# deepmarkpy/aware

Hardware: AMD Instinct MI355X
Metric: waveform-seconds/sec through embed->attack->detect; BER vs reference (higher is better)
Workload: dtype f32 accumulation on the 16-bit MFMA pipe; conv-block GEMMs: every f32 operand scaled by a power of two and carried as TWO binary16 terms (within one f32 ulp of the operand, rms 2^-24.5), 3 partial products, the l_a*l_b term (<= 2^-22) dropped -- gemm_h2.hip: error level of an f32 dot product (agains

## Files before the change

### aware_amd/_lib.py

```python
from __future__ import annotations

import ctypes as C
import glob
import os
import subprocess

_HERE = os.path.dirname(os.path.abspath(__file__))
LIB_PATH = os.environ.get("AWARE_HIP_LIB") or os.path.join(_HERE, "libaware_hip.so")
CSRC = os.path.join(_HERE, "csrc")
SOURCES = ["capi.hip", "dsp_kernels.hip", "dsp_stream.hip", "seam_kernels.hip", "detector_kernels.hip", "gemm_x3.hip", "gemm_h2.hip", "attack_kernels.hip", "stft_any.hip", "loop_any.hip", "stoi_kernels.hip", "loop_attack_kernels.hip", "loop_reverb_kernels.hip", "loop_speed_kernels.hip", "loop_stretch_kernels.hip", "loop_pitch_kernels.hip", "loop_pv_kernels.hip", "loop_delete_kernels.hip", "loop_filter_kernels.hip", "sync_kernels.hip", "loop_mix_kernels.hip", "loop_gain_kernels.hip", "speed_search_kernels.hip", "scan_kernels.hip", "viterbi_kernels.hip"]

AWARE_OK = 0
ERRORS = {-1: "bad argument", -2: "unsupported configuration", -3: "HIP runtime error", -4: "workspace too small"}


class AwareHipError(RuntimeError):
    pass


def build_library(force: bool = False, verbose: bool = False) -> str:
    from concurrent.futures import ThreadPoolExecutor
    hdrs = glob.glob(os.path.join(CSRC, "*.hpp")) + glob.glob(os.path.join(CSRC, "*.h")) + [
        os.path.join(_HERE, "..", "include", "aware_hip.h")]
    hdr_t = max(os.path.getmtime(h) for h in hdrs)
# ... 135 lines not shown
    "aware_opt_clamp_step": (_i, [_i, _vp, _vp, _vp, _vp, _vp, _vp, _sz, C.POINTER(C.c_float), C.POINTER(C.c_float), _vp]),
    "aware_embed_begin": (_i, [_vp, _vp, _vp, _vp]),
    "aware_embed_iterate": (_i, [_vp, _i, _vp]),
    "aware_embed_profile": (_i, [_vp, _i, _i, _vp, _vp, _vp]),
    "aware_embed_gradient": (_i, [_vp, _vp, _vp]),
    "aware_embed_finish": (_i, [_vp, _vp, _vp, _vp]),
    "aware_embed_buffer": (_vp, [_vp, _i]),
    "aware_pcm_quantize": (_i, [_vp, _vp, _vp, _vp, _i, _i, _i, _vp, _vp]),
    "aware_waveform_normalize": (_i, [_vp, _vp, _vp, _vp, _i, _i, _vp, _vp]),
    "aware_upfirdn": (_i, [_vp, _vp, _vp, _vp, _vp, _vp, _i, _i, _vp, _i, _i, _i, _i, _vp]),
    "aware_iir": (_i, [_vp, _vp, _vp, _i, _i, _vp, _i, _vp, _vp, _vp, _i, _i, _vp, _vp]),
    "aware_decimate_interp": (_i, [_vp, _vp, _vp, _i, _i, _i, _vp, _vp]),
    "aware_segment_cut": (_i, [_vp, _vp, _vp, _vp, _vp, _vp, _vp, _i, _i, _i, _vp]),
    "aware_phase_vocoder": (_i, [_vp, _vp, _vp, _vp, _i, C.c_double, _vp]),
    "aware_snr": (_i, [_vp, _vp, _vp, _vp, _vp, _i, _vp, _vp]),
    "aware_stoi_create": (_i, [C.POINTER(_vp)]),
    "aware_stoi_destroy": (None, [_vp]),
    "aware_stoi_band_edges": (_i, [_vp, _pi, _pi]),
    "aware_stoi_frames": (_i, [_i]),
    "aware_stoi_workspace_bytes": (_sz, [_i, _i, C.c_longlong]),
    "aware_stoi": (_i, [_vp, _vp, _vp, _vp, _vp, _vp, _i, _i, C.c_longlong, _vp, _vp, _vp, _sz, _vp]),
    "aware_gaussian_noise": (_i, [_vp, _vp, _vp, _vp, _i, _i, _vp, _f, _vp, _vp]),
    "aware_spectral_quantize": (_i, [_vp, _i, _f, _f, _vp]),
    "aware_spectral_quantize_bwd": (_i, [_vp, _vp, _vp, _i, _f, _f, _vp]),
    "aware_gemm_nt_variant": (_i, [_vp, _i, _vp, _i, _vp, _vp, _i, _i, _i, _i, _i, _vp]),
    "aware_x3_packed_bytes": (_sz, [_i, _i]),
    "aware_x3_pack": (_i, [_vp, _i, _i, _vp]),
    "aware_gemm_clip": (_i, [_vp, _i, _vp, _i, _vp, _vp, _vp, _i, _i, _i, _i, _i, _i, _vp, _vp, _i, _vp]),
    "aware_gemm_clip_last": (_i, [_vp, _i, _vp, _vp, _vp, _i, _i, _i, _i, _i, _vp, _vp, _vp, _i, _vp]),
    "aware_gemm_clip_h2_workspace_bytes": (_sz, [_i, _i, _i]),
    "aware_gemm_clip_h2": (_i, [_vp, _i, _vp, _i, _vp, _vp, _i, _i, _i, _i, _i, _i, _vp, _vp, _vp, _vp, _i, _vp, _vp, _sz, _vp]),
    "aware_gemm_clip_h2_tile": (_i, [_vp, _i, _vp, _i, _vp, _vp, _i, _i, _i, _i, _i, _i, _vp, _vp, _vp, _vp, _i, _vp, _vp, _sz, _i,
                                     _vp]),
    "aware_gemm_nt": (_i, [_vp, _i, _vp, _i, _vp, _vp, _i, _i, _i, _i, _vp]),
}

_lib = None


def load_library():
    global _lib
    if _lib is not None:
        return _lib
    if not os.path.exists(LIB_PATH):
        raise AwareHipError(
            f"{LIB_PATH} is missing: build it with `python -c 'import __graft_entry__ as g; g.build()'` "
            "(hipcc --offload-arch=gfx950).  aware_amd has no CPU fallback.")
    import torch
    lib = C.CDLL(LIB_PATH)
    for name, (res, args) in SIGNATURES.items():
        fn = getattr(lib, name)
        fn.restype = res
        fn.argtypes = args
    _lib = lib
    return lib


def check(rc: int, what: str = ""):
    if rc != AWARE_OK:
        lib = load_library()
        detail = lib.aware_last_hip_error().decode() if rc == -3 else ""
        raise AwareHipError(f"{what}: {ERRORS.get(rc, rc)} {detail}".strip())


def require_gpu():
    import torch
# ... 4 lines not shown
```

### aware_amd/csrc/capi.hip

```cpp
#include <hip/hip_runtime.h>
#include <math.h>
#include <cmath>
#include <stdio.h>
#include <stdlib.h>
#include <string.h>
#include <string>
#include <algorithm>
#include <vector>

#include "../../include/aware_hip.h"
#include "common.hpp"
#include "kernels.h"
#define AWARE_LOOP_CF cf
#include "loop_chain.hpp"

using namespace aware;

static thread_local std::string g_last_err;

#define HIPCHK(expr)                                                                  \
    do {                                                                              \
        hipError_t _e = (expr);                                                       \
        if (_e != hipSuccess) {                                                       \
            g_last_err = std::string(#expr) + ": " + hipGetErrorString(_e);           \
// ... 2923 lines not shown

extern "C" size_t aware_gemm_clip_h2_workspace_bytes(int B, int N, int K) {
    return (B > 0 && N > 0 && K > 0) ? h2_packed_bytes(N, K) + (size_t)B * 64 * sizeof(float) * 2 + 1024 : 0;
}
extern "C" int aware_gemm_clip_h2(const float* A, int lda, const float* Bt, int ldb, const float* bias, float* C, int ldc, int B,
                                  int Tp, int N, int K, int epi, float* rstd_io, const float* act, const void* lastpk, float* zpart,
                                  int CL, float* amax_out, void* workspace, size_t workspace_bytes, void* stream) {
    return aware_gemm_clip_h2_tile(A, lda, Bt, ldb, bias, C, ldc, B, Tp, N, K, epi, rstd_io, act, lastpk, zpart, CL, amax_out,
                                   workspace, workspace_bytes, 0, stream);
}
extern "C" int aware_gemm_clip_h2_tile(const float* A, int lda, const float* Bt, int ldb, const float* bias, float* C, int ldc,
                                       int B, int Tp, int N, int K, int epi, float* rstd_io, const float* act, const void* lastpk,
                                       float* zpart, int CL, float* amax_out, void* workspace, size_t workspace_bytes, int tile,
                                       void* stream) {
    if (tile < 0 || tile > 2) return AWARE_E_BADARG;
    if (!A || !Bt || !C || !workspace || B < 1 || Tp < 1 || Tp > 128 || epi < 0 || epi > 2 || (ldb & 3)) return AWARE_E_BADARG;
    if (epi != 0 && !rstd_io) return AWARE_E_BADARG;
    if (epi == 2 && !act) return AWARE_E_BADARG;
    const int nwm = (Tp + 31) / 32;
    if (!gemm_clip_h2_supported(nwm, N, K, lda) || N % 16) return AWARE_E_BADARG;
    if (tile == 2 && !gemm_clip_h2_wide_supported(nwm, N, K, lda)) return AWARE_E_UNSUPPORTED;
    if (workspace_bytes < aware_gemm_clip_h2_workspace_bytes(B, N, K)) return AWARE_E_WORKSPACE;
    hipStream_t st = (hipStream_t)stream;
    Carver c(workspace, workspace_bytes);
    void* pk = c.take<char>(h2_packed_bytes(N, K));
    float* amax = c.take<float>((size_t)B * 64);
    launch_h2_pack(Bt, ldb, N, K, pk, st);
    launch_clip_amax(A, lda, K, 32 * nwm, B, amax, st);
    launch_gemm_clip_h2(A, lda, pk, amax, amax_out, bias, C, ldc, B, nwm, Tp, N, K, epi, rstd_io, act, st,
                        (epi == 1 && lastpk && zpart) ? lastpk : nullptr, zpart, CL, tile == 2 ? 2 : 1);
    LAUNCHCHK();
    return AWARE_OK;
}

extern "C" int aware_gemm_nt(const float* A, int lda, const float* Bt, int ldb, const float* bias, float* C, int ldc,
                             int M, int N, int K, void* stream) {
    if (!A || !Bt || !C || M < 1 || N < 1 || K < 4 || (K & 3) || (lda & 3) || (ldb & 3)) return AWARE_E_BADARG;
    launch_gemm_nt(A, lda, Bt, ldb, bias, C, ldc, M, N, K, (hipStream_t)stream);
    LAUNCHCHK();
    return AWARE_OK;
}
```

### aware_amd/csrc/conv_block.hpp

```cpp
#pragma once
#include <hip/hip_runtime.h>
#include "split_bf16.hpp"

namespace aware {

constexpr int kConvFrag = 1024;

template <class P, int RG, int EPI>
constexpr int conv_block_lds_bytes() {
    constexpr int stage = 2 * 2 * P::kTerms * 2 * RG * kConvFrag;
    constexpr int last = 32 * RG * 132 * 4 > 8 * RG * 3 * kConvFrag ? 32 * RG * 132 * 4 : 8 * RG * 3 * kConvFrag;
    return (EPI == X3_FWD_LAST && last > stage) ? last : stage;
}

constexpr int conv_tile_width(int NT, int NW) { return 16 * NT * NW; }

__host__ __device__ inline int conv_slab_group(int tiles_n, int width, int K, int weight_bytes) {
    int sg = (int)(3355443u / (unsigned)(width * K * weight_bytes));
    sg = sg < 1 ? 1 : (sg > tiles_n ? tiles_n : sg);
    while (tiles_n % sg) --sg;
    return sg;
}

template <class P, int RG, int EPI, int NT = 1, int NW = 8>
__device__ __forceinline__ void conv_block_uniform(const float* __restrict__ A, int lda, const u32x4* __restrict__ Bpk,
                                                   const float* __restrict__ binv, const float* __restrict__ amax_in,
                                                   float* __restrict__ amax_out, const float* __restrict__ bias,
                                                   float* __restrict__ C, int ldc, int Tp, int N, int K, int tiles_n, int ntiles,
                                                   float* __restrict__ rstd_io, const float* __restrict__ act,
                                                   const u32x4* __restrict__ Lpk, float* __restrict__ zpart, int CL, int Mrows) {
    constexpr int MT = 2 * RG;
    constexpr int MH = RG;
    constexpr int FRAG = kConvFrag;
    constexpr int W = conv_tile_width(NT, NW);
    static_assert(NT == 1 || P::kScaled, "the row-major PLAIN epilogue of the unscaled format is written for one column tile");
    static_assert(W % 128 == 0 && (NW == 8 || NW == 4), "FWD_LAST works on whole 128-column slabs with 4 or 8 waves");
    __shared__ __attribute__((aligned(16))) unsigned char lds[conv_block_lds_bytes<P, RG, EPI>()];

    int id = blockIdx.x;
    int clip, slab;
    if ((ntiles & 7) == 0) {
        const int x = id & 7, j = id >> 3, R = ntiles >> 3;
        const int nclip = R / tiles_n;
        if (nclip * tiles_n == R && nclip > 0) {
            const int sg = conv_slab_group(tiles_n, W, K, P::kWeightBytes);
            const int per_group = nclip * sg;
            const int grp = j / per_group, r = j % per_group;
            clip = x * nclip + r / sg;
            slab = grp * sg + r % sg;
        } else {
            id = x * R + j;
            clip = id / tiles_n;
            slab = id % tiles_n;
        }
    } else {
        clip = id / tiles_n;
        slab = id % tiles_n;
    }
    const int bm = clip * 32 * RG;
    const int bn = slab * W;
    const int tid = threadIdx.x, lane = tid & 63, wave = tid >> 6;
    const int r16 = lane & 15, kg = lane >> 4;
    const int col0 = bn + wave * (16 * NT) + r16;

    float ascale = 1.f, ainv = 1.f;
    if constexpr (P::kScaled) {
        float am = lane < (K >> 4) ? amax_in[(size_t)clip * 64 + lane] : 0.f;
#pragma unroll
        for (int o = 32; o > 0; o >>= 1) am = fmaxf(am, __shfl_xor(am, o));
        ascale = __uint_as_float(__builtin_amdgcn_readfirstlane(__float_as_uint(P::scale_for(am))));
    }

    f32x4 acc[MT][NT];
    const int row_limit = (!P::kScaled && EPI == X3_PLAIN) ? min(32 * RG, Mrows - bm) : 32 * RG;
    if constexpr (NT == 1 && NW == 8) P::template tile_gemm<RG>(A, lda, Bpk, K, bm, bn, lds, acc, row_limit, ascale);
    else P::template tile_gemm<RG, NT, NW>(A, lda, Bpk, K, bm, bn, lds, acc, row_limit, ascale);

    if constexpr (P::kScaled) ainv = P::pow2_inverse(ascale);
    const float invT = 1.0f / (float)Tp;
    if constexpr (!P::kScaled && EPI == X3_PLAIN) {
        if ((ldc & 3) == 0) {
            float (*T)[132] = reinterpret_cast<float (*)[132]>(lds);
            const float bv = bias ? bias[col0] : 0.f;
            __syncthreads();
#pragma unroll
            for (int m = 0; m < MT; ++m)
#pragma unroll
                for (int e = 0; e < 4; ++e) T[16 * m + 4 * kg + e][16 * wave + r16] = acc[m][0][e] + bv;
            __syncthreads();
            const int c4 = (lane & 31) * 4, rr = 2 * wave + (lane >> 5);
#pragma unroll
            for (int j = 0; j < MT; ++j) {
                const int row = rr + 16 * j;
                float4 o = *reinterpret_cast<const float4*>(&T[row][c4]);
                if (row >= Tp) o = make_float4(0.f, 0.f, 0.f, 0.f);
                if (bm + row < Mrows) *reinterpret_cast<float4*>(C + (size_t)(bm + row) * ldc + bn + c4) = o;
            }
            return;
        }
    }
#pragma unroll
    for (int n = 0; n < NT; ++n) {
    const int col = col0 + 16 * n;
    float bcol = 1.f;
    if constexpr (P::kScaled) bcol = binv[col];
    float omax = 0.f;
    if (EPI == X3_PLAIN) {
        const float bv = bias ? bias[col] : 0.f;
#pragma unroll
        for (int m = 0; m < MT; ++m)
#pragma unroll
            for (int e = 0; e < 4; ++e) {
                const int row = m * 16 + 4 * kg + e;
                const float o = row < Tp ? fmaf(acc[m][n][e] * ainv, bcol, bv) : 0.f;
                omax = fmaxf(omax, fabsf(o));
                if (P::kScaled || bm + row < Mrows) C[(size_t)(bm + row) * ldc + col] = o;
            }
    } else if (EPI == X3_FWD || EPI == X3_FWD_LAST) {
        const float bv = bias ? bias[col] : 0.f;
        float s = 0.f;
#pragma unroll
        for (int m = 0; m < MT; ++m)
#pragma unroll
            for (int e = 0; e < 4; ++e) {
                const int row = m * 16 + 4 * kg + e;
                acc[m][n][e] = fmaf(acc[m][n][e] * ainv, bcol, bv);
                if (row < Tp) s += acc[m][n][e];
            }
        s += __shfl_xor(s, 16);
        s += __shfl_xor(s, 32);
        const float mean = s * invT;
        auto centre = [&](float x) {
            if constexpr (P::kScaled) return fmaf(-invT, s, x);
            else return x - mean;
        };
        float qq = 0.f;
#pragma unroll
        for (int m = 0; m < MT; ++m)
#pragma unroll
            for (int e = 0; e < 4; ++e) {
                const int row = m * 16 + 4 * kg + e;
                if (row < Tp) {
                    const float d = centre(acc[m][n][e]);
                    if constexpr (P::kScaled) qq = fmaf(d, d, qq);
                    else qq += d * d;
                }
            }
        qq += __shfl_xor(qq, 16);
        qq += __shfl_xor(qq, 32);
        const float rs = 1.0f / sqrtf(qq * invT + 1e-5f);
        if (kg == 0) rstd_io[(size_t)clip * N + col] = rs;
#pragma unroll
        for (int m = 0; m < MT; ++m)
#pragma unroll
            for (int e = 0; e < 4; ++e) {
                const int row = m * 16 + 4 * kg + e;
                const float u = centre(acc[m][n][e]) * rs;
                const float o = row < Tp ? (u > 0.f ? u : 0.2f * u) : 0.f;
                acc[m][n][e] = o;
                omax = fmaxf(omax, fabsf(o));
                C[(size_t)(bm + row) * ldc + col] = o;
            }
    } else {
        const float rs = rstd_io[(size_t)clip * N + col];
        float s1 = 0.f, s2 = 0.f;
        float u[MT][4];
#pragma unroll
        for (int m = 0; m < MT; ++m)
#pragma unroll
            for (int e = 0; e < 4; ++e) {
                const int row = m * 16 + 4 * kg + e;
                const float av = act[(size_t)(bm + row) * ldc + col];
                const bool valid = row < Tp;
                const float uv = valid ? (av > 0.f ? av : av * 5.0f) : 0.f;
                const float du = valid ? acc[m][n][e] * ainv * bcol * (av > 0.f ? 1.f : 0.2f) : 0.f;
                acc[m][n][e] = du;
                u[m][e] = uv;
                s1 += du;
                s2 += du * uv;
            }
        s1 += __shfl_xor(s1, 16);
        s1 += __shfl_xor(s1, 32);
        s2 += __shfl_xor(s2, 16);
        s2 += __shfl_xor(s2, 32);
        const float m1 = s1 * invT, m2 = s2 * invT;
#pragma unroll
        for (int m = 0; m < MT; ++m)
#pragma unroll
            for (int e = 0; e < 4; ++e) {
                const int row = m * 16 + 4 * kg + e;
                const float o = row < Tp ? rs * (acc[m][n][e] - m1 - u[m][e] * m2) : 0.f;
                omax = fmaxf(omax, fabsf(o));
                C[(size_t)(bm + row) * ldc + col] = o;
            }
    }
    if constexpr (P::kScaled) {
        if (amax_out) {
#pragma unroll
            for (int o = 32; o > 0; o >>= 1) omax = fmaxf(omax, __shfl_xor(omax, o));
            if (lane == 0) amax_out[(size_t)clip * 64 + (col >> 4)] = omax;
        }
    }
    }
    if (EPI == X3_FWD_LAST) {
        const int KS2L = N >> 5, ncl = (CL + 15) >> 4;
        constexpr int UH = 8 / NW;
        constexpr int WS = 8 / NT;
        const int tq = NW == 8 ? wave >> 1 : wave, mh0 = NW == 8 ? wave & 1 : 0;
        float* const T = reinterpret_cast<float*>(lds);
        constexpr int TP = 132;
#pragma unroll
        for (int sl = 0; sl < W / 128; ++sl) {
        const int slab128 = (bn >> 7) + sl;
        bf16x8 bl[3][3];
#pragma unroll
        for (int n = 0; n < 3; ++n)
            if (n < ncl) {
#pragma unroll
                for (int p = 0; p < 3; ++p)
                    bl[n][p] = __builtin_bit_cast(bf16x8, Lpk[(((size_t)n * KS2L + 4 * slab128 + tq) * 3 + p) * 64 + lane]);
            }
        __syncthreads();
        if (wave / WS == sl) {
#pragma unroll
            for (int n = 0; n < NT; ++n)
#pragma unroll
                for (int m = 0; m < MT; ++m)
#pragma unroll
                    for (int e = 0; e < 4; ++e)
                        T[(16 * m + 4 * kg + e) * TP + 16 * ((wave % WS) * NT + n) + r16] = acc[m][n][e];
        }
        __syncthreads();
        f32x4 zt[UH * MH][3];
#pragma unroll
        for (int mm = 0; mm < UH * MH; ++mm) {
#pragma unroll
            for (int n = 0; n < 3; ++n) zt[mm][n] = f32x4{0.f, 0.f, 0.f, 0.f};
            const float* src = T + (16 * (mh0 * MH + mm) + r16) * TP + 32 * tq + 8 * kg;
            const float4 x0 = *reinterpret_cast<const float4*>(src), x1 = *reinterpret_cast<const float4*>(src + 4);
            uint4 q0, q1, q2;
            split_pair(x0.x, x0.y, q0.x, q1.x, q2.x);
            split_pair(x0.z, x0.w, q0.y, q1.y, q2.y);
            split_pair(x1.x, x1.y, q0.z, q1.z, q2.z);
            split_pair(x1.z, x1.w, q0.w, q1.w, q2.w);
            bf16x8 a[3];
            a[0] = __builtin_bit_cast(bf16x8, q0); a[1] = __builtin_bit_cast(bf16x8, q1); a[2] = __builtin_bit_cast(bf16x8, q2);
#pragma unroll
            for (int term = 0; term < 6; ++term) {
                const int pa = term == 0 ? 2 : (term == 1 || term == 3) ? 1 : 0;
                const int pb = term == 2 ? 2 : (term == 1 || term == 4) ? 1 : 0;
#pragma unroll
                for (int n = 0; n < 3; ++n)
                    if (n < ncl) zt[mm][n] = __builtin_amdgcn_mfma_f32_16x16x32_bf16(a[pa], bl[n][pb], zt[mm][n], 0, 0, 0);
            }
        }
        __syncthreads();
#pragma unroll
        for (int mm = 0; mm < UH * MH; ++mm)
#pragma unroll
            for (int n = 0; n < 3; ++n)
                *reinterpret_cast<f32x4*>(lds + (size_t)((tq * MT + mh0 * MH + mm) * 3 + n) * FRAG + lane * 16) = zt[mm][n];
        __syncthreads();
        for (int rt = wave; rt < MT; rt += NW) {
            float* zp = zpart + (size_t)slab128 * ((size_t)(ntiles / tiles_n) * 32 * RG * CL) + (size_t)(bm + 16 * rt + 4 * kg) * CL;
#pragma unroll
// ... 298 lines not shown
```

### aware_amd/csrc/gemm_h2.hip

```cpp
#include <hip/hip_runtime.h>
#include <stdint.h>
#include "kernels.h"
#include "common.hpp"
#include "split_bf16.hpp"
#include "conv_block.hpp"

namespace aware {

typedef _Float16 f16x8 __attribute__((ext_vector_type(8)));
typedef _Float16 f16x2 __attribute__((ext_vector_type(2)));

static inline size_t h2_plane_bytes(int N, int K) { return (size_t)N * (size_t)(((K + 31) / 32) * 32) * 2 * sizeof(uint16_t); }
size_t h2_packed_bytes(int N, int K) { return h2_plane_bytes(N, K) + (size_t)N * sizeof(float); }
const float* h2_inv_scale(const void* packed, int N, int K) { return (const float*)((const char*)packed + h2_plane_bytes(N, K)); }

__device__ __forceinline__ float h2_scale_for(float amax) {
    const int e = (int)((__float_as_uint(amax) >> 23) & 0xFFu);
    return __uint_as_float((unsigned)(267 - max(e, 14)) << 23);
}
__device__ __forceinline__ float h2_pow2_inverse(float s) {
    const unsigned e = (__float_as_uint(s) >> 23) & 0xFFu;
    return __uint_as_float((254u - e) << 23);
}

// ... 161 lines not shown
            H2_PIN(0x008, MH * NT);
            if (q == 3) {
                lds_barrier();
                read_h(0, noff);
                H2_PIN(0x100, MH);
            }
            read_l(noff);
            H2_PIN(0x100, MH);
            __builtin_amdgcn_s_setprio(1);
            H2_MFMA(ah[q & 1], bq[t][1], hf);
            H2_MFMA(ah[q & 1], bq[t][0], hf);
            H2_PIN(0x008, 2 * MH * NT);
            __builtin_amdgcn_s_setprio(0);
        }
    }
#undef H2_PIN
#undef H2_MFMA
}

struct H2Ops {
    static constexpr bool kScaled = true;
    static constexpr int kWeightBytes = 4;
    static constexpr int kTerms = 2;
    template <int RG, int NT = 1, int NW = 8>
    __device__ static __forceinline__ void tile_gemm(const float* __restrict__ A, int lda, const u32x4* __restrict__ Bpk, int K,
                                                     int bm, int bn, unsigned char* lds, f32x4 (&acc)[2 * RG][NT], int row_limit,
                                                     float ascale) {
        h2_tile_gemm<RG, NT, NW>(A, lda, Bpk, K, bm, bn, lds, acc, row_limit, ascale);
    }
    __device__ static __forceinline__ float scale_for(float amax) { return h2_scale_for(amax); }
    __device__ static __forceinline__ float pow2_inverse(float s) { return h2_pow2_inverse(s); }
};

template <int RG, int EPI, int NT = 1, int NW = 8>
__global__ __launch_bounds__(64 * NW, NT > 1 ? 2 : RG <= 3 ? 4 : 2) void gemm_clip_h2_kernel(
    const float* __restrict__ A, int lda, const u32x4* __restrict__ Bpk, const float* __restrict__ binv,
    const float* __restrict__ amax_in, float* __restrict__ amax_out, const float* __restrict__ bias, float* __restrict__ C, int ldc,
    int Tp, int N, int K, int tiles_n, int ntiles, float* __restrict__ rstd_io, const float* __restrict__ act,
    const u32x4* __restrict__ Lpk, float* __restrict__ zpart, int CL) {
    conv_block_uniform<H2Ops, RG, EPI, NT, NW>(A, lda, Bpk, binv, amax_in, amax_out, bias, C, ldc, Tp, N, K, tiles_n, ntiles, rstd_io,
                                               act, Lpk, zpart, CL, 0);
}

template <int EPI>
__global__ __launch_bounds__(512, 4) void gemm_ragged_h2_kernel(const float* __restrict__ A, int lda, const u32x4* __restrict__ Bpk,
                                                                const float* __restrict__ binv, const float* __restrict__ amax_in,
                                                                float* __restrict__ amax_out, const float* __restrict__ bias,
                                                                float* __restrict__ C, int ldc, const int* __restrict__ frame_off,
                                                                const int* __restrict__ pool_off, const int* __restrict__ order, int N,
                                                                int K, int tiles_n, int ntiles, float* __restrict__ rstd_io,
                                                                const float* __restrict__ act) {
    conv_block_ragged<H2Ops, EPI>(A, lda, Bpk, binv, amax_in, amax_out, bias, C, ldc, frame_off, pool_off, order, N, K, tiles_n,
                                  ntiles, rstd_io, act);
}

void launch_gemm_ragged_h2(const float* A, int lda, const void* Bpk, const float* amax_in, float* amax_out, const float* bias,
                           float* C, int ldc, int B, const int* frame_off, const int* pool_off, const int* order, int N, int K,
                           int epi, float* rstd_io, const float* act, hipStream_t st) {
    const int tn = N / 128;
    const float* binv = h2_inv_scale(Bpk, N, K);
    constexpr size_t kLds = ragged_lds_bytes<H2Ops>();
    if (epi == X3_FWD)
        hipLaunchKernelGGL((gemm_ragged_h2_kernel<X3_FWD>), dim3(tn * B), dim3(512), kLds, st, A, lda, (const u32x4*)Bpk, binv, amax_in,
                           amax_out, bias, C, ldc, frame_off, pool_off, order, N, K, tn, tn * B, rstd_io, act);
    else
        hipLaunchKernelGGL((gemm_ragged_h2_kernel<X3_BWD>), dim3(tn * B), dim3(512), kLds, st, A, lda, (const u32x4*)Bpk, binv, amax_in,
                           amax_out, bias, C, ldc, frame_off, pool_off, order, N, K, tn, tn * B, rstd_io, act);
}

__global__ __launch_bounds__(256) void ragged_amax_kernel(const float* __restrict__ A, int lda, int K, const int* __restrict__ frame_off,
                                                           const int* __restrict__ pool_off, float* __restrict__ amax) {
    __shared__ float red[4];
    const int clip = blockIdx.x, tid = threadIdx.x;
    const int Tp = (frame_off[clip + 1] - frame_off[clip]) / 2, row0 = pool_off[clip];
    const int k4 = K >> 2;
    float m = 0.f;
    for (int i = tid; i < Tp * k4; i += 256) {
        const int r = i / k4, c = i % k4;
        const float4 v = *reinterpret_cast<const float4*>(A + (size_t)(row0 + r) * lda + 4 * c);
        m = fmaxf(fmaxf(m, fmaxf(fabsf(v.x), fabsf(v.y))), fmaxf(fabsf(v.z), fabsf(v.w)));
    }
#pragma unroll
    for (int o = 32; o > 0; o >>= 1) m = fmaxf(m, __shfl_xor(m, o));
    if ((tid & 63) == 0) red[tid >> 6] = m;
    __syncthreads();
    const int np = K >> 4;
    if (tid < np) amax[(size_t)clip * 64 + tid] = tid == 0 ? fmaxf(fmaxf(red[0], red[1]), fmaxf(red[2], red[3])) : 0.f;
}
void launch_ragged_amax(const float* A, int lda, int K, const int* frame_off, const int* pool_off, int B, float* amax, hipStream_t st) {
    hipLaunchKernelGGL(ragged_amax_kernel, dim3(B), dim3(256), 0, st, A, lda, K, frame_off, pool_off, amax);
}

bool gemm_clip_h2_supported(int nwm, int N, int K, int lda) {
    return nwm >= 1 && nwm <= 4 && N % 128 == 0 && K % 64 == 0 && K <= 1024 && lda % 4 == 0;
}
bool gemm_clip_h2_wide_supported(int nwm, int N, int K, int lda) {
    return gemm_clip_h2_supported(nwm, N, K, lda) && nwm <= 3 && N % kH2WideTile == 0;
}


void launch_gemm_clip_h2(const float* A, int lda, const void* Bpk, const float* amax_in, float* amax_out, const float* bias,
                         float* C, int ldc, int B, int nwm, int Tp, int N, int K, int epi, float* rstd_io, const float* act,
                         hipStream_t st, const void* lastpk, float* zpart, int CL, int tile) {
    const float* binv = h2_inv_scale(Bpk, N, K);
    if (epi == X3_FWD && lastpk && zpart) epi = X3_FWD_LAST;
    const bool wide = tile == 2 && nwm <= 3;
    const int tn = N / (wide ? kH2WideTile : 128);
#define HK(M_, E_, NT_, NW_) hipLaunchKernelGGL((gemm_clip_h2_kernel<M_, E_, NT_, NW_>), dim3(tn * B), dim3(64 * NW_), 0, st, A, lda, \
                                                (const u32x4*)Bpk, binv, amax_in, amax_out, bias, C, ldc, Tp, N, K, tn, tn * B,        \
                                                rstd_io, act, (const u32x4*)lastpk, zpart, CL)
#define HM(E_)                                                                                                                 \
    if (wide) switch (nwm) { case 1: HK(1, E_, 4, 4); break; case 2: HK(2, E_, 4, 4); break; default: HK(3, E_, 4, 4); break; }  \
    else switch (nwm) { case 1: HK(1, E_, 1, 8); break; case 2: HK(2, E_, 1, 8); break; case 3: HK(3, E_, 1, 8); break;          \
                        default: HK(4, E_, 1, 8); break; }
    if (epi == X3_FWD) { HM(X3_FWD) } else if (epi == X3_BWD) { HM(X3_BWD) } else if (epi == X3_FWD_LAST) { HM(X3_FWD_LAST) }
    else { HM(X3_PLAIN) }
#undef HM
#undef HK
}

}
```

### aware_amd/csrc/kernels.h

```cpp
#pragma once
#include <hip/hip_runtime.h>
#include <stddef.h>
#include <stdint.h>
#include "common.hpp"
#include "loop_limits.hpp"

namespace aware {

struct LoopMixDrawLaunch {
    const unsigned* seeds = nullptr;
    const int* step = nullptr;
    int step_imm = 0, B = 0, n = 0;
    unsigned long long thr[kMaxLoopChains] = {0};
    int* choice = nullptr;
};
void launch_loop_mix_draw(const LoopMixDrawLaunch& L, hipStream_t st);

constexpr int kStreamWaves = 4;

struct AnalysisLaunch {
    PlanDev plan;
    const int* frame_off = nullptr;
    int B = 0, max_frames = 0;
    int run_frames = 0, n_wg = 0;
// ... 77 lines not shown
void launch_oob_residual(const float* audio, const int* in_off, const unsigned long long* pmax, const int* pcount,
                         int pstride, const float* band, const int* frame_off, float* oob, int B, int max_frames,
                         hipStream_t st);
void launch_finish(const float* yraw, const int* frame_off, const unsigned long long* pmax, const int* pcount,
                   int pstride, const float* rescale, float* out, const int* out_off, int B, int max_frames,
                   hipStream_t st);

void launch_gemm_nt(const float* A, int lda, const float* Bt, int ldb, const float* bias, float* C, int ldc, int M,
                    int N, int K, hipStream_t st);
void launch_gemm_nt_variant(const float* A, int lda, const float* Bt, int ldb, const float* bias, float* C, int ldc,
                            int M, int N, int K, int variant, hipStream_t st);
int gemm_autotune(const float* A, int lda, const float* Bt, int ldb, float* C, int ldc, int M, int N, int K,
                  hipStream_t st);
void launch_gemm_clip(const float* A, int lda, const float* Bt, int ldb, const float* bias, float* C, int ldc, int B,
                      int nwm, int Tp, int N, int K, int epi, float* rstd_io, const float* act, hipStream_t st);
size_t x3_packed_bytes(int N, int K);
void x3_pack(const float* Wt, int N, int K, uint16_t* out);
void launch_x3_pack_dev(const float* Wt_dev, int ldw, int Nvalid, int Kvalid, int N, int K, void* out, hipStream_t st);
bool gemm_clip_x3_supported(int nwm, int N, int K, int lda);
bool mel_front_x3_supported(int T, int K, int lda);
void launch_mel_front_x3(const float* mag, int lda, const void* melTpk, const int* frame_off, const int* pool_off, float* xm,
                         float* x0, float* stats, float* gstat, int B, int T, int K, hipStream_t st, float* amax_out = nullptr);
void launch_mel_back_x3(const float* dZ, int lda, const void* wTpk, const int* frame_off, const int* pool_off, float* xm,
                        const float* stats, const float* gstat, int B, int T, int K, hipStream_t st);
void launch_gemm_clip_x3(const float* A, int lda, const void* Bpk, const float* bias, float* C, int ldc, int B, int nwm,
                         int Tp, int N, int K, int epi, float* rstd_io, const float* act, hipStream_t st,
                         const void* lastpk = nullptr, float* zpart = nullptr, int CL = 0, int Mrows = 0);
size_t h2_packed_bytes(int N, int K);
void launch_h2_pack(const float* Wt_dev, int ldw, int N, int K, void* out, hipStream_t st);
void launch_clip_amax(const float* A, int lda, int K, int rows_per_clip, int B, float* amax, hipStream_t st);
bool gemm_clip_h2_supported(int nwm, int N, int K, int lda);
constexpr int kH2WideTile = 256;
bool gemm_clip_h2_wide_supported(int nwm, int N, int K, int lda);
void launch_gemm_clip_h2(const float* A, int lda, const void* Bpk, const float* amax_in, float* amax_out, const float* bias,
                         float* C, int ldc, int B, int nwm, int Tp, int N, int K, int epi, float* rstd_io, const float* act,
                         hipStream_t st, const void* lastpk = nullptr, float* zpart = nullptr, int CL = 0, int tile = 1);
void launch_gemm_ragged_h2(const float* A, int lda, const void* Bpk, const float* amax_in, float* amax_out, const float* bias,
                           float* C, int ldc, int B, const int* frame_off, const int* pool_off, const int* order, int N, int K,
                           int epi, float* rstd_io, const float* act, hipStream_t st);
void launch_ragged_amax(const float* A, int lda, int K, const int* frame_off, const int* pool_off, int B, float* amax, hipStream_t st);
void launch_gemm_ragged_x3(const float* A, int lda, const void* Bpk, const float* bias, float* C, int ldc, int B,
                           const int* frame_off, const int* pool_off, const int* order, int N, int K, int epi, float* rstd_io,
                           const float* act, hipStream_t st);
bool readout_x3_supported(int nwm, int ci, int C);
void launch_readout_x3(const float* hin, int ci, const float* zpart, int nslab, const float* bias, const void* WTpk,
                       const float* rstd_prev, const float* target, float* pred, float* loss, float* best_loss, int* improved,
                       int* step, float* dZ, int B, int nwm, int Tp, int C, int nbits, int loss_kind, hipStream_t st,
                       const float* loss_add, void* img, float* amax_out = nullptr);
size_t readout_x3_image_bytes(int B, int nwm);
void launch_readout_grad_ragged_x3(const float* hin, int ci, const float* dZl, const void* WTpk, const float* rstd_prev, float* dZ,
                                   const int* frame_off, const int* pool_off, const int* order, int B, hipStream_t st,
                                   float* amax_out = nullptr);
constexpr int kMelClipFrames = 192;
void launch_mel_norm_fwd(const float* xm, const int* frame_off, const int* pool_off, float* x0, float* stats, float* gstat,
                         float* part, int pstride, int B, int max_frames, int n_mels, int Mp, hipStream_t st,
                         float* amax_out = nullptr);
void launch_mel_norm_bwd(const float* dx0, float* xm_inout, const int* frame_off, const int* pool_off, const float* stats,
                         const float* gstat, float* part, int pstride, int B, int max_frames, int n_mels, int Mp, hipStream_t st);
void launch_in_lrelu_fwd(float* z, const int* frame_off, const int* pool_off, float* rstd, int C, int B, int max_pooled,
                         hipStream_t st);
void launch_in_lrelu_bwd(float* dA, const float* A, const int* frame_off, const int* pool_off, const float* rstd, int C, int B,
                         int max_pooled, hipStream_t st);
constexpr int kActRelu = 0, kActLRelu = 1, kActGelu = 2, kActSwish = 3, kActTanh = 4, kActSigmoid = 5;
constexpr int kNormInstance = 0, kNormAffine = 1, kNormNone = 2;
AW_HD bool norm_act_needs_stash(int norm, int act) {
    return !(act == kActLRelu || (act == kActRelu && norm != kNormInstance));
// ... 334 lines not shown
```

### aware_amd/runtime.py

```python
from __future__ import annotations

import ctypes as C
import math
from typing import Sequence

import numpy as np
import torch

from . import _lib
from ._lib import AwareHipError, DetectorArch, EmbedConfig, check, load_library, require_gpu

SPEC_STRIDE = 256
SPEC_STRIDE_WIDE = 576
FULL_STRIDE = 520
CONV_PIPES = {"f16x2": 0, "f32": 1, "bf16x3": 2}
CONV_TILES = {"auto": 0, "narrow": 1, "wide": 2}
LOSS_KINDS = {"push_extremes": 0, "mse": 1, "hinge": 2, "sign": 3, "push_sigmoid": 4, "ber": 5, "push_extremes_l1": 6}


def band_stride(band_lo: int, band_hi: int) -> int:
    return SPEC_STRIDE if band_lo >= 1 and band_hi <= 511 and band_hi - band_lo + 1 <= SPEC_STRIDE else SPEC_STRIDE_WIDE


def general_band_stride(nband: int) -> int:
# ... 676 lines not shown
    check(lib.aware_gemm_nt(_ptr(a), a.stride(0), _ptr(bt), bt.stride(0), _ptr(bias), _ptr(c), N, M, N, K, _stream()),
          "aware_gemm_nt")
    return c


def x3_pack(wt: torch.Tensor) -> torch.Tensor:
    lib = load_library()
    w = np.ascontiguousarray(wt.detach().cpu().numpy(), dtype=np.float32)
    N, K = w.shape
    nbytes = int(lib.aware_x3_packed_bytes(N, K))
    if nbytes == 0:
        raise AwareHipError("aware_x3_pack: N must be a positive multiple of 16")
    out = np.zeros(nbytes, dtype=np.uint8)
    check(lib.aware_x3_pack(w.ctypes.data, N, K, out.ctypes.data), "aware_x3_pack")
    return torch.from_numpy(out).cuda()


def gemm_clip(a: torch.Tensor, bt: torch.Tensor, bias, B: int, Tp: int, epi: int = 0, rstd=None, act=None,
              mode: int = 0, packed=None):
    lib = load_library()
    M, K = a.shape
    N = bt.shape[0]
    c = torch.empty((M, N), dtype=torch.float32, device=a.device)
    if rstd is None:
        rstd = torch.zeros((B, N), dtype=torch.float32, device=a.device)
    if mode == 1 and packed is None:
        packed = x3_pack(bt)
    check(lib.aware_gemm_clip(_ptr(a), a.stride(0), _ptr(bt), bt.stride(0), _ptr(packed), _ptr(bias), _ptr(c), N, B, Tp, N, K,
                              epi, _ptr(rstd), _ptr(act), mode, _stream()), "aware_gemm_clip")
    return c, rstd


def gemm_clip_h2(a: torch.Tensor, bt: torch.Tensor, bias, B: int, Tp: int, epi: int = 0, rstd=None, act=None, w_last=None,
                 tile: int = 0):
    lib = load_library()
    M, K = a.shape
    N = bt.shape[0]
    dev = a.device
    btd = bt.to(dev).contiguous()
    c = torch.empty((M, N), dtype=torch.float32, device=dev)
    if rstd is None:
        rstd = torch.zeros((B, N), dtype=torch.float32, device=dev)
    amax = torch.zeros((B, 64), dtype=torch.float32, device=dev)
    nbytes = int(lib.aware_gemm_clip_h2_workspace_bytes(B, N, K))
    ws = torch.empty(nbytes, dtype=torch.uint8, device=dev)
    pkl, zpart, CL = None, None, 0
    if w_last is not None:
        CL = w_last.shape[0]
        wl = torch.zeros((16 * ((CL + 15) // 16), N), dtype=torch.float32)
        wl[:CL] = w_last.detach().cpu().float()
        pkl = x3_pack(wl)
        zpart = torch.zeros((N // 128, M, CL), dtype=torch.float32, device=dev)
    check(lib.aware_gemm_clip_h2_tile(_ptr(a), a.stride(0), _ptr(btd), btd.stride(0), _ptr(bias), _ptr(c), N, B, Tp, N, K, epi,
                                      _ptr(rstd), _ptr(act), _ptr(pkl), _ptr(zpart), CL, _ptr(amax), _ptr(ws), nbytes, int(tile),
                                      _stream()), "aware_gemm_clip_h2_tile")
    torch.cuda.current_stream().synchronize()
    return (c, rstd, amax) if w_last is None else (c, rstd, amax, zpart)


def gemm_clip_last(a: torch.Tensor, bt: torch.Tensor, bias, w_last: torch.Tensor, B: int, Tp: int):
    lib = load_library()
    M, K = a.shape
    N = bt.shape[0]
    CL = w_last.shape[0]
    clp = 16 * ((CL + 15) // 16)
    wl = torch.zeros((clp, N), dtype=torch.float32)
    wl[:CL] = w_last.detach().cpu().float()
    c = torch.empty((M, N), dtype=torch.float32, device=a.device)
    rstd = torch.zeros((B, N), dtype=torch.float32, device=a.device)
    zpart = torch.zeros((N // 128, M, CL), dtype=torch.float32, device=a.device)
    pk, pkl = x3_pack(bt), x3_pack(wl)
    check(lib.aware_gemm_clip_last(_ptr(a), a.stride(0), _ptr(pk), _ptr(bias), _ptr(c), N, B, Tp, N, K, _ptr(rstd),
                                   _ptr(pkl), _ptr(zpart), CL, _stream()), "aware_gemm_clip_last")
    torch.cuda.current_stream().synchronize()
    return c, rstd, zpart


class Ragged:

    def __init__(self, data: torch.Tensor, lengths: Sequence[int]):
        self.data = data
        self.lengths = [int(n) for n in lengths]
        self.offsets = np.concatenate([[0], np.cumsum(self.lengths)[:-1]]).astype(np.int64).tolist()
        self.B = len(self.lengths)
        self.max_len = max(self.lengths)
        dev = data.device
        self.d_off = torch.tensor(self.offsets, dtype=torch.int32, device=dev)
        self.d_len = torch.tensor(self.lengths, dtype=torch.int32, device=dev)

    @classmethod
# ... 557 lines not shown
```

### include/aware_hip.h

```cpp
#ifndef AWARE_HIP_H
#define AWARE_HIP_H

#include <stddef.h>
#include <stdint.h>

#ifdef __cplusplus
extern "C" {
#endif

#define AWARE_OK 0
#define AWARE_E_BADARG (-1)
#define AWARE_E_UNSUPPORTED (-2)
#define AWARE_E_HIP (-3)
#define AWARE_E_WORKSPACE (-4)

#define AWARE_LOSS_PUSH_EXTREMES 0
#define AWARE_LOSS_MSE 1
#define AWARE_LOSS_HINGE 2
#define AWARE_LOSS_SIGN 3
#define AWARE_LOSS_PUSH_SIGMOID 4
#define AWARE_LOSS_BER 5
#define AWARE_LOSS_PUSH_L1 6
#define AWARE_LOSS_EXTERNAL 7

// ... 257 lines not shown

int aware_speed_views(const float* in, const int* in_off, const int* in_len, int B, const int* m, int n_views, float* out,
                      const int* out_off, int max_len, void* stream);

int aware_scan_select(const float* values, const int* win_off, int B, int n_sync, int L, float centre, float* win_conf,
                      int* win_view, float* win_values, uint32_t* win_bits, void* stream);
int aware_scan_segments(const float* win_conf, const int* win_view, const float* win_values, const uint32_t* win_bits,
                        const int* win_off, const int* win_off_dev, int B, int L, float centre, float min_confidence,
                        int max_flip, int max_segments, int* n_seg, int* seg_first, int* seg_last, int* seg_peak,
                        int* seg_view, float* seg_conf, float* seg_values, void* stream);

int aware_viterbi_decode(const float* values, int R, int L, float centre, int rate_n, int crc_bits, uint32_t* bits,
                         float* metric, int* valid, int* corrected, void* stream);

int aware_gemm_nt(const float* A, int lda, const float* Bt, int ldb, const float* bias, float* C, int ldc,
                  int M, int N, int K, void* stream);
int aware_gemm_nt_variant(const float* A, int lda, const float* Bt, int ldb, const float* bias, float* C, int ldc,
                          int M, int N, int K, int variant, void* stream);

size_t aware_x3_packed_bytes(int N, int K);
int aware_x3_pack(const float* host_wt, int N, int K, void* host_out);
int aware_gemm_clip(const float* A, int lda, const float* Bt, int ldb, const void* Bpk, const float* bias, float* C,
                    int ldc, int B, int Tp, int N, int K, int epi, float* rstd_io, const float* act, int mode,
                    void* stream);
int aware_gemm_clip_last(const float* A, int lda, const void* Bpk, const float* bias, float* C, int ldc, int B, int Tp,
                         int N, int K, float* rstd_out, const void* lastpk, float* zpart, int CL, void* stream);
size_t aware_gemm_clip_h2_workspace_bytes(int B, int N, int K);
int aware_gemm_clip_h2(const float* A, int lda, const float* Bt, int ldb, const float* bias, float* C, int ldc, int B, int Tp,
                       int N, int K, int epi, float* rstd_io, const float* act, const void* lastpk, float* zpart, int CL,
                       float* amax_out, void* workspace, size_t workspace_bytes, void* stream);
int aware_gemm_clip_h2_tile(const float* A, int lda, const float* Bt, int ldb, const float* bias, float* C, int ldc, int B,
                            int Tp, int N, int K, int epi, float* rstd_io, const float* act, const void* lastpk, float* zpart,
                            int CL, float* amax_out, void* workspace, size_t workspace_bytes, int tile, void* stream);

#ifdef __cplusplus
}
#endif
#endif
```

Baseline: 2000.

## Stage wide-tile conv GEMM epilogue through LDS for row-major vectorised stores

For the wide (NT=4, NW=4) h2 conv-block kernel, the epilogue now stages each wave's MFMA accumulator fragments through a swizzled LDS region. It then writes C, and reads the activation input in the backward epilogue, as row-contiguous float4 accesses instead of strided scalar accesses. The FWD_LAST path reuses its existing transpose buffer to emit float4 rows. A form selector picks this path only when C and act are 16-byte aligned. This adds LDS traffic and wave-level barriers, plus a block sync before the epilogue, in exchange for coalesced global memory access.

```diff
diff --git a/aware_amd/_lib.py b/aware_amd/_lib.py
--- a/aware_amd/_lib.py
+++ b/aware_amd/_lib.py
@@ -191,6 +191,7 @@
     "aware_gemm_clip_h2": (_i, [_vp, _i, _vp, _i, _vp, _vp, _i, _i, _i, _i, _i, _i, _vp, _vp, _vp, _vp, _i, _vp, _vp, _sz, _vp]),
     "aware_gemm_clip_h2_tile": (_i, [_vp, _i, _vp, _i, _vp, _vp, _i, _i, _i, _i, _i, _i, _vp, _vp, _vp, _vp, _i, _vp, _vp, _sz, _i,
                                      _vp]),
+    "aware_gemm_clip_h2_form": (_i, [_vp, _i, _vp, _i, _i, _i, _i, _i, _i, _i]),
     "aware_gemm_nt": (_i, [_vp, _i, _vp, _i, _vp, _vp, _i, _i, _i, _i, _vp]),
 }
 
diff --git a/aware_amd/csrc/capi.hip b/aware_amd/csrc/capi.hip
--- a/aware_amd/csrc/capi.hip
+++ b/aware_amd/csrc/capi.hip
@@ -2979,6 +2979,14 @@
     LAUNCHCHK();
     return AWARE_OK;
 }
+extern "C" int aware_gemm_clip_h2_form(const float* C, int ldc, const float* act, int Tp, int N, int K, int lda, int epi, int last,
+                                       int tile) {
+    if (tile < 0 || tile > 2 || !C || Tp < 1 || Tp > 128 || epi < 0 || epi > 2) return AWARE_E_BADARG;
+    const int nwm = (Tp + 31) / 32;
+    if (!gemm_clip_h2_supported(nwm, N, K, lda) || N % 16) return AWARE_E_BADARG;
+    if (tile == 2 && !gemm_clip_h2_wide_supported(nwm, N, K, lda)) return AWARE_E_UNSUPPORTED;
+    return gemm_clip_h2_form(tile == 2 ? 2 : 1, nwm, epi, last != 0, C, ldc, act);
+}
 
 extern "C" int aware_gemm_nt(const float* A, int lda, const float* Bt, int ldb, const float* bias, float* C, int ldc,
                              int M, int N, int K, void* stream) {
diff --git a/aware_amd/csrc/conv_block.hpp b/aware_amd/csrc/conv_block.hpp
--- a/aware_amd/csrc/conv_block.hpp
+++ b/aware_amd/csrc/conv_block.hpp
@@ -1,6 +1,7 @@
 #pragma once
 #include <hip/hip_runtime.h>
 #include "split_bf16.hpp"
+#include "conv_epilogue_rows.hpp"
 
 namespace aware {
 
@@ -22,7 +23,7 @@
     return sg;
 }
 
-template <class P, int RG, int EPI, int NT = 1, int NW = 8>
+template <class P, int RG, int EPI, int NT = 1, int NW = 8, bool ROWS = false>
 __device__ __forceinline__ void conv_block_uniform(const float* __restrict__ A, int lda, const u32x4* __restrict__ Bpk,
                                                    const float* __restrict__ binv, const float* __restrict__ amax_in,
                                                    float* __restrict__ amax_out, const float* __restrict__ bias,
@@ -35,6 +36,7 @@
     constexpr int W = conv_tile_width(NT, NW);
     static_assert(NT == 1 || P::kScaled, "the row-major PLAIN epilogue of the unscaled format is written for one column tile");
     static_assert(W % 128 == 0 && (NW == 8 || NW == 4), "FWD_LAST works on whole 128-column slabs with 4 or 8 waves");
+    static_assert(!ROWS || (NT == 4 && NW == 4 && P::kScaled), "the row-major epilogue is written for the wide form");
     __shared__ __attribute__((aligned(16))) unsigned char lds[conv_block_lds_bytes<P, RG, EPI>()];
 
     int id = blockIdx.x;
@@ -99,8 +101,39 @@
             return;
         }
     }
+    namespace er = epi_rows;
+    constexpr int RJ = ROWS ? er::row_passes(RG) : 1;
+    constexpr bool kTurn = ROWS && EPI != X3_FWD_LAST;
+    float* const reg = reinterpret_cast<float*>(lds) + wave * er::region_floats(RG);
+    auto wave_sync = [&]() {
+        __builtin_amdgcn_fence(__ATOMIC_RELEASE, "wavefront");
+        __builtin_amdgcn_wave_barrier();
+        __builtin_amdgcn_fence(__ATOMIC_ACQUIRE, "wavefront");
+    };
+    auto half_offset = [&](int h, int j) {
+        return (size_t)(bm + er::rm_row(lane, j)) * ldc + (bn + wave * (16 * NT) + 32 * h + er::rm_col(lane));
+    };
+    f32x4 ar[2][RJ];
+    auto load_act = [&](int h) {
+#pragma unroll
+        for (int j = 0; j < RJ; ++j) ar[h][j] = *reinterpret_cast<const f32x4*>(act + half_offset(h, j));
+    };
+    if constexpr (kTurn) {
+        if constexpr (EPI == X3_BWD) {
+            load_act(0);
+            load_act(1);
+        }
+        __syncthreads();
+    }
 #pragma unroll
     for (int n = 0; n < NT; ++n) {
+    if constexpr (kTurn && EPI == X3_BWD) {
+        if ((n & 1) == 0) {
+#pragma unroll
+            for (int j = 0; j < RJ; ++j) *reinterpret_cast<f32x4*>(reg + er::act_write(lane, j)) = ar[n >> 1][j];
+            wave_sync();
+        }
+    }
     const int col = col0 + 16 * n;
     float bcol = 1.f;
     if constexpr (P::kScaled) bcol = binv[col];
@@ -114,7 +147,8 @@
                 const int row = m * 16 + 4 * kg + e;
                 const float o = row < Tp ? fmaf(acc[m][n][e] * ainv, bcol, bv) : 0.f;
                 omax = fmaxf(omax, fabsf(o));
-                if (P::kScaled || bm + row < Mrows) C[(size_t)(bm + row) * ldc + col] = o;
+                if constexpr (ROWS) acc[m][n][e] = o;
+                else if (P::kScaled || bm + row < Mrows) C[(size_t)(bm + row) * ldc + col] = o;
             }
     } else if (EPI == X3_FWD || EPI == X3_FWD_LAST) {
         const float bv = bias ? bias[col] : 0.f;
@@ -159,7 +193,7 @@
                 const float o = row < Tp ? (u > 0.f ? u : 0.2f * u) : 0.f;
                 acc[m][n][e] = o;
                 omax = fmaxf(omax, fabsf(o));
-                C[(size_t)(bm + row) * ldc + col] = o;
+                if constexpr (!ROWS) C[(size_t)(bm + row) * ldc + col] = o;
             }
     } else {
         const float rs = rstd_io[(size_t)clip * N + col];
@@ -170,7 +204,9 @@
 #pragma unroll
             for (int e = 0; e < 4; ++e) {
                 const int row = m * 16 + 4 * kg + e;
-                const float av = act[(size_t)(bm + row) * ldc + col];
+                float av;
+                if constexpr (ROWS) av = reg[er::act_read(lane, m, n & 1, e)];
+                else av = act[(size_t)(bm + row) * ldc + col];
                 const bool valid = row < Tp;
                 const float uv = valid ? (av > 0.f ? av : av * 5.0f) : 0.f;
                 const float du = valid ? acc[m][n][e] * ainv * bcol * (av > 0.f ? 1.f : 0.2f) : 0.f;
@@ -191,8 +227,22 @@
                 const int row = m * 16 + 4 * kg + e;
                 const float o = row < Tp ? rs * (acc[m][n][e] - m1 - u[m][e] * m2) : 0.f;
                 omax = fmaxf(omax, fabsf(o));
-                C[(size_t)(bm + row) * ldc + col] = o;
-            }
+                if constexpr (ROWS) acc[m][n][e] = o;
+                else C[(size_t)(bm + row) * ldc + col] = o;
+            }
+    }
+    if constexpr (kTurn) {
+#pragma unroll
+        for (int m = 0; m < MT; ++m)
+#pragma unroll
+            for (int e = 0; e < 4; ++e) reg[er::c_write(lane, m, n & 1, e)] = acc[m][n][e];
+        if (n & 1) {
+            wave_sync();
+#pragma unroll
+            for (int j = 0; j < RJ; ++j)
+                *reinterpret_cast<float4*>(C + half_offset(n >> 1, j)) = *reinterpret_cast<const float4*>(reg + er::c_read(lane, j));
+            wave_sync();
+        }
     }
     if constexpr (P::kScaled) {
         if (amax_out) {
@@ -231,6 +281,15 @@
                         T[(16 * m + 4 * kg + e) * TP + 16 * ((wave % WS) * NT + n) + r16] = acc[m][n][e];
         }
         __syncthreads();
+        if constexpr (ROWS) {
+            const int c4 = (lane & 31) * 4, rr = 2 * wave + (lane >> 5);
+#pragma unroll
+            for (int j = 0; j < 4 * RG; ++j) {
+                const int row = rr + 8 * j;
+                *reinterpret_cast<float4*>(C + (size_t)(bm + row) * ldc + bn + 128 * sl + c4) =
+                    *reinterpret_cast<const float4*>(T + row * TP + c4);
+            }
+        }
         f32x4 zt[UH * MH][3];
 #pragma unroll
         for (int mm = 0; mm < UH * MH; ++mm) {
diff --git a/aware_amd/csrc/conv_epilogue_rows.hpp b/aware_amd/csrc/conv_epilogue_rows.hpp
--- /dev/null
+++ b/aware_amd/csrc/conv_epilogue_rows.hpp
@@ -0,0 +1,28 @@
+#pragma once
+#if defined(__HIPCC__) || defined(__CUDACC__)
+#define AWARE_HD __host__ __device__
+#else
+#define AWARE_HD
+#endif
+
+namespace aware {
+namespace epi_rows {
+
+constexpr int kCols = 32;
+AWARE_HD constexpr int region_floats(int RG) { return 32 * RG * kCols; }
+AWARE_HD constexpr int row_passes(int RG) { return 4 * RG; }
+
+AWARE_HD inline int slot(int row, int col) { return row * kCols + (col ^ (((row >> 2) & 1) << 4)); }
+
+AWARE_HD inline int acc_row(int lane, int m, int e) { return 16 * m + 4 * (lane >> 4) + e; }
+AWARE_HD inline int acc_col(int lane, int nl) { return 16 * nl + (lane & 15); }
+AWARE_HD inline int rm_row(int lane, int j) { return 8 * j + (lane >> 3); }
+AWARE_HD inline int rm_col(int lane) { return 4 * (lane & 7); }
+
+AWARE_HD inline int c_write(int lane, int m, int nl, int e) { return slot(acc_row(lane, m, e), acc_col(lane, nl)); }
+AWARE_HD inline int c_read(int lane, int j) { return slot(rm_row(lane, j), rm_col(lane)); }
+AWARE_HD inline int act_write(int lane, int j) { return slot(rm_row(lane, j), rm_col(lane)); }
+AWARE_HD inline int act_read(int lane, int m, int nl, int e) { return slot(acc_row(lane, m, e), acc_col(lane, nl)); }
+
+}
+}
diff --git a/aware_amd/csrc/gemm_h2.hip b/aware_amd/csrc/gemm_h2.hip
--- a/aware_amd/csrc/gemm_h2.hip
+++ b/aware_amd/csrc/gemm_h2.hip
@@ -217,14 +217,14 @@
     __device__ static __forceinline__ float pow2_inverse(float s) { return h2_pow2_inverse(s); }
 };
 
-template <int RG, int EPI, int NT = 1, int NW = 8>
+template <int RG, int EPI, int NT = 1, int NW = 8, bool ROWS = false>
 __global__ __launch_bounds__(64 * NW, NT > 1 ? 2 : RG <= 3 ? 4 : 2) void gemm_clip_h2_kernel(
     const float* __restrict__ A, int lda, const u32x4* __restrict__ Bpk, const float* __restrict__ binv,
     const float* __restrict__ amax_in, float* __restrict__ amax_out, const float* __restrict__ bias, float* __restrict__ C, int ldc,
     int Tp, int N, int K, int tiles_n, int ntiles, float* __restrict__ rstd_io, const float* __restrict__ act,
     const u32x4* __restrict__ Lpk, float* __restrict__ zpart, int CL) {
-    conv_block_uniform<H2Ops, RG, EPI, NT, NW>(A, lda, Bpk, binv, amax_in, amax_out, bias, C, ldc, Tp, N, K, tiles_n, ntiles, rstd_io,
-                                               act, Lpk, zpart, CL, 0);
+    conv_block_uniform<H2Ops, RG, EPI, NT, NW, ROWS>(A, lda, Bpk, binv, amax_in, amax_out, bias, C, ldc, Tp, N, K, tiles_n, ntiles,
+                                                     rstd_io, act, Lpk, zpart, CL, 0);
 }
 
 template <int EPI>
@@ -284,23 +284,38 @@
 }
 
 
+#ifndef AWARE_H2_ROW_EPILOGUES
+#define AWARE_H2_ROW_EPILOGUES ((1 << X3_PLAIN) | (1 << X3_FWD) | (1 << X3_BWD) | (1 << X3_FWD_LAST))
+#endif
+constexpr int kH2RowEpilogues = AWARE_H2_ROW_EPILOGUES;
+
+int gemm_clip_h2_form(int tile, int nwm, int epi, bool last, const float* C, int ldc, const float* act) {
+    if (tile != 2 || nwm > 3) return 1;
+    if (epi == X3_FWD && last) epi = X3_FWD_LAST;
+    const bool aligned = (ldc & 3) == 0 && ((uintptr_t)C & 15) == 0 && (epi != X3_BWD || ((uintptr_t)act & 15) == 0);
+    return aligned && ((kH2RowEpilogues >> epi) & 1) ? 3 : 2;
+}
+
 void launch_gemm_clip_h2(const float* A, int lda, const void* Bpk, const float* amax_in, float* amax_out, const float* bias,
                          float* C, int ldc, int B, int nwm, int Tp, int N, int K, int epi, float* rstd_io, const float* act,
                          hipStream_t st, const void* lastpk, float* zpart, int CL, int tile) {
     const float* binv = h2_inv_scale(Bpk, N, K);
+    const int form = gemm_clip_h2_form(tile, nwm, epi, lastpk && zpart, C, ldc, act);
     if (epi == X3_FWD && lastpk && zpart) epi = X3_FWD_LAST;
-    const bool wide = tile == 2 && nwm <= 3;
+    const bool wide = form >= 2, rows = form == 3;
     const int tn = N / (wide ? kH2WideTile : 128);
-#define HK(M_, E_, NT_, NW_) hipLaunchKernelGGL((gemm_clip_h2_kernel<M_, E_, NT_, NW_>), dim3(tn * B), dim3(64 * NW_), 0, st, A, lda, \
-                                                (const u32x4*)Bpk, binv, amax_in, amax_out, bias, C, ldc, Tp, N, K, tn, tn * B,        \
-                                                rstd_io, act, (const u32x4*)lastpk, zpart, CL)
+#define HK(M_, E_, NT_, NW_, R_) hipLaunchKernelGGL((gemm_clip_h2_kernel<M_, E_, NT_, NW_, R_>), dim3(tn * B), dim3(64 * NW_), 0, st, \
+                                                    A, lda, (const u32x4*)Bpk, binv, amax_in, amax_out, bias, C, ldc, Tp, N, K, tn,    \
+                                                    tn * B, rstd_io, act, (const u32x4*)lastpk, zpart, CL)
+#define HW(M_, E_) if (rows) HK(M_, E_, 4, 4, true); else HK(M_, E_, 4, 4, false)
 #define HM(E_)                                                                                                                 \
-    if (wide) switch (nwm) { case 1: HK(1, E_, 4, 4); break; case 2: HK(2, E_, 4, 4); break; default: HK(3, E_, 4, 4); break; }  \
-    else switch (nwm) { case 1: HK(1, E_, 1, 8); break; case 2: HK(2, E_, 1, 8); break; case 3: HK(3, E_, 1, 8); break;          \
-                        default: HK(4, E_, 1, 8); break; }
+    if (wide) switch (nwm) { case 1: HW(1, E_); break; case 2: HW(2, E_); break; default: HW(3, E_); break; }                    \
+    else switch (nwm) { case 1: HK(1, E_, 1, 8, false); break; case 2: HK(2, E_, 1, 8, false); break;                            \
+                        case 3: HK(3, E_, 1, 8, false); break; default: HK(4, E_, 1, 8, false); break; }
     if (epi == X3_FWD) { HM(X3_FWD) } else if (epi == X3_BWD) { HM(X3_BWD) } else if (epi == X3_FWD_LAST) { HM(X3_FWD_LAST) }
     else { HM(X3_PLAIN) }
 #undef HM
+#undef HW
 #undef HK
 }
 
diff --git a/aware_amd/csrc/kernels.h b/aware_amd/csrc/kernels.h
--- a/aware_amd/csrc/kernels.h
+++ b/aware_amd/csrc/kernels.h
@@ -133,6 +133,7 @@
 bool gemm_clip_h2_supported(int nwm, int N, int K, int lda);
 constexpr int kH2WideTile = 256;
 bool gemm_clip_h2_wide_supported(int nwm, int N, int K, int lda);
+int gemm_clip_h2_form(int tile, int nwm, int epi, bool last, const float* C, int ldc, const float* act);
 void launch_gemm_clip_h2(const float* A, int lda, const void* Bpk, const float* amax_in, float* amax_out, const float* bias,
                          float* C, int ldc, int B, int nwm, int Tp, int N, int K, int epi, float* rstd_io, const float* act,
                          hipStream_t st, const void* lastpk = nullptr, float* zpart = nullptr, int CL = 0, int tile = 1);
diff --git a/aware_amd/runtime.py b/aware_amd/runtime.py
--- a/aware_amd/runtime.py
+++ b/aware_amd/runtime.py
@@ -732,13 +732,21 @@
 
 
 def gemm_clip_h2(a: torch.Tensor, bt: torch.Tensor, bias, B: int, Tp: int, epi: int = 0, rstd=None, act=None, w_last=None,
-                 tile: int = 0):
+                 tile: int = 0, out=None):
     lib = load_library()
     M, K = a.shape
     N = bt.shape[0]
     dev = a.device
     btd = bt.to(dev).contiguous()
-    c = torch.empty((M, N), dtype=torch.float32, device=dev)
+    if out is None:
+        c = torch.empty((M, N), dtype=torch.float32, device=dev)
+    else:
+        c = out
+        if tuple(c.shape) != (M, N) or c.stride(1) != 1 or c.stride(0) < N or c.dtype != torch.float32 or c.device != dev:
+            raise ValueError("out: an [M, N] f32 view on a's device with unit column stride and a row pitch of at least N")
+    ldc = c.stride(0)
+    if act is not None and (act.stride(0) != ldc or act.stride(1) != 1):
+        raise ValueError("act: the row pitch of C")
     if rstd is None:
         rstd = torch.zeros((B, N), dtype=torch.float32, device=dev)
     amax = torch.zeros((B, 64), dtype=torch.float32, device=dev)
@@ -751,11 +759,19 @@
         wl[:CL] = w_last.detach().cpu().float()
         pkl = x3_pack(wl)
         zpart = torch.zeros((N // 128, M, CL), dtype=torch.float32, device=dev)
-    check(lib.aware_gemm_clip_h2_tile(_ptr(a), a.stride(0), _ptr(btd), btd.stride(0), _ptr(bias), _ptr(c), N, B, Tp, N, K, epi,
+    check(lib.aware_gemm_clip_h2_tile(_ptr(a), a.stride(0), _ptr(btd), btd.stride(0), _ptr(bias), _ptr(c), ldc, B, Tp, N, K, epi,
                                       _ptr(rstd), _ptr(act), _ptr(pkl), _ptr(zpart), CL, _ptr(amax), _ptr(ws), nbytes, int(tile),
                                       _stream()), "aware_gemm_clip_h2_tile")
     torch.cuda.current_stream().synchronize()
     return (c, rstd, amax) if w_last is None else (c, rstd, amax, zpart)
+
+
+def gemm_clip_h2_form(c: torch.Tensor, act, Tp: int, K: int, epi: int = 0, last: bool = False, tile: int = 0) -> int:
+    lib = load_library()
+    rc = int(lib.aware_gemm_clip_h2_form(_ptr(c), c.stride(0), _ptr(act), Tp, c.shape[1], K, K, epi, int(last), int(tile)))
+    if rc < 0:
+        check(rc, "aware_gemm_clip_h2_form")
+    return rc
 
 
 def gemm_clip_last(a: torch.Tensor, bt: torch.Tensor, bias, w_last: torch.Tensor, B: int, Tp: int):
diff --git a/include/aware_hip.h b/include/aware_hip.h
--- a/include/aware_hip.h
+++ b/include/aware_hip.h
@@ -313,6 +313,7 @@
 int aware_gemm_clip_h2_tile(const float* A, int lda, const float* Bt, int ldb, const float* bias, float* C, int ldc, int B,
                             int Tp, int N, int K, int epi, float* rstd_io, const float* act, const void* lastpk, float* zpart,
                             int CL, float* amax_out, void* workspace, size_t workspace_bytes, int tile, void* stream);
+int aware_gemm_clip_h2_form(const float* C, int ldc, const float* act, int Tp, int N, int K, int lda, int epi, int last, int tile);
 
 #ifdef __cplusplus
 }
```

Result: faster. 2053, median of 6 (+2.6%).
